# omarezz46/BayesDLL

Hardware: AMD Instinct MI355X
Metric: SG-HMC leapfrog steps/sec & HBM GB/s on ViT-L/32 params, 1/2/4/8 MI355X (higher is better)
Workload: dtype f32

## Files before the change

bayesdll_amd/_lib.py:

```python
from __future__ import annotations

import ctypes as C
import os
import threading

import numpy as np
import torch

HERE = os.path.dirname(os.path.abspath(__file__))
LIB_PATH = os.environ.get("BDL_SGMCMC_LIB", os.path.join(HERE, "libbdl_sgmcmc.so"))

BDL_OK = 0
CSGHMC, SGHMC, SGLD, SGHMC_GRAD, SGLD_GRAD, ADAM_SGHMC, ADAM_SGHMC_GRAD = range(7)
NOISE_NONE, NOISE_BUFFER, NOISE_PHILOX = 0, 1, 2
COLLECT_NONE, COLLECT_WELFORD_INIT, COLLECT_WELFORD, COLLECT_MEAN_INIT, COLLECT_MEAN = range(5)
MIX_BARE, MIX_PIPELINED, MIX_PACED = 0, 1, 2
ATTR_HEAD, ATTR_PRIOR, ATTR_SKIP, ATTR_GUNALIGNED = 0x1, 0x2, 0x4, 0x8
FLAG_FIRST_STEP, FLAG_RECIP_DIV, FLAG_MOMENTUM, FLAG_GRAD_READY = 0x1, 0x2, 0x4, 0x8
VAR_GIVEN, VAR_RAW_MOMENTS, VAR_WELFORD = 0, 1, 2
ABI_VERSION = 8

_fp = C.c_void_p


# ... 363 lines not shown


class MemberScore(C.Structure):
    _fields_ = [("n", C.c_int64), ("n_nonfinite", C.c_int64), ("n_wrong", C.c_int64),
                ("nll_sum", C.c_double)]


class MemberScoreArgs(C.Structure):
    _fields_ = [("logits", _fp), ("labels", _fp), ("scores", _fp), ("workspace", _fp),
                ("batch", C.c_int64), ("members", C.c_int32), ("groups", C.c_int32),
                ("classes", C.c_int32), ("grid_blocks", C.c_int32), ("flags", C.c_int32),
                ("pad0", C.c_int32)]


class MixtureTotals(C.Structure):
    _fields_ = [("n", C.c_int64), ("n_nonfinite", C.c_int64),
                ("expected_entropy_sum", C.c_double)]


class MixtureArgs(C.Structure):
    _fields_ = [("logits", _fp), ("weights", _fp), ("labels", _fp), ("logp", _fp),
                ("expected_entropy", _fp), ("totals", _fp), ("workspace", _fp),
                ("batch", C.c_int64), ("components", C.c_int32), ("draws", C.c_int32),
                ("groups", C.c_int32), ("classes", C.c_int32), ("combine", C.c_int32),
                ("grid_blocks", C.c_int32), ("flags", C.c_int32), ("pad0", C.c_int32)]


MIXTURE_EXPORTS = {
    "bdl_member_score_workspace_bytes": (C.c_int64, [C.c_int32, C.c_int32, C.c_int32]),
    "bdl_mixture_workspace_bytes": (C.c_int64, [C.c_int32, C.c_int32]),
    "bdl_member_score": (C.c_int, [C.POINTER(MemberScoreArgs), C.c_void_p]),
    "bdl_mixture": (C.c_int, [C.POINTER(MixtureArgs), C.c_void_p]),
}

RANK_U, RANK_ITILE, RANK_JTILE, RANK_MAX_ROWS = 2, 512, 1024, 65535
RANK_MAX_N = 2 ** 31 - 1


class RankTotals(C.Structure):
    _fields_ = [("n_pos", C.c_int64), ("n_neg", C.c_int64), ("n_excluded", C.c_int64),
                ("u2", C.c_int64), ("fp_at_tpr", C.c_int64), ("ap_sum", C.c_double)]


class RankArgs(C.Structure):
    _fields_ = [("scores", _fp), ("marks", _fp), ("ge_pos", _fp), ("ge_neg", _fp),
                ("gt_neg", _fp), ("totals", _fp), ("workspace", _fp), ("n", C.c_int64),
                ("need", C.c_int64), ("rows", C.c_int32), ("scores_per_group", C.c_int32),
                ("mark_rows", C.c_int32), ("tpr_num", C.c_int32), ("tpr_den", C.c_int32),
                ("pad0", C.c_int32)]


RANK_EXPORTS = {
    "bdl_rank_workspace_bytes": (C.c_int64, [C.c_int32, C.c_int64]),
    "bdl_rank": (C.c_int, [C.POINTER(RankArgs), C.c_void_p]),
}

DIVERSITY_MAX_VOTERS, DIVERSITY_MAX_CLASSES, DIVERSITY_WAVE_VOTERS = 64, 8192, 16
DIVERSITY_TILE, DIVERSITY_LDS_STRIDE, DIVERSITY_MAX_GRID = 64, 68, 1024
DIVERSITY_DEFAULT_WORKSPACE = 32 << 20
DIVERSITY_RESET = 0x1
DIVERSITY_INT_MATRICES = ("disagree", "both_wrong", "kl_unbounded")
DIVERSITY_SUM_MATRICES = ("tv_sum", "kl_sum")


def diversity_totals_dtype(voters):
    P = int(voters)
    return np.dtype([(k, np.int64) for k in ("n", "n_labelled", "n_nonfinite", "voters")]
                    + [(k, np.int64, (P, P)) for k in DIVERSITY_INT_MATRICES]
                    + [(k, np.float64, (P, P)) for k in DIVERSITY_SUM_MATRICES])


class DiversityArgs(C.Structure):
    _fields_ = [("logits", _fp), ("labels", _fp), ("totals", _fp), ("workspace", _fp),
                ("batch", C.c_int64), ("voters", C.c_int32), ("classes", C.c_int32),
                ("grid_blocks", C.c_int32), ("flags", C.c_int32)]


DIVERSITY_EXPORTS = {
    "bdl_diversity_totals_bytes": (C.c_int64, [C.c_int32]),
    "bdl_diversity_workspace_bytes": (C.c_int64, [C.c_int32, C.c_int32]),
    "bdl_diversity": (C.c_int, [C.POINTER(DiversityArgs), C.c_void_p]),
}

_lib = None
_lock = threading.Lock()


def lib():
    global _lib
    if _lib is not None:
        return _lib
    with _lock:
        if _lib is None:
            if not os.path.exists(LIB_PATH):
                raise RuntimeError(
                    f"bayesdll_amd: HIP library not found at {LIB_PATH}; build it with "
                    "`make -C bayesdll_amd/csrc` (or __graft_entry__.build()). There is no CPU "
                    "fallback for the fused SG-MCMC step.")
            h = C.CDLL(LIB_PATH)
            for name, (res, argt) in (list(EXPORTS.items()) + list(DIAG_EXPORTS.items())
                                      + list(CLIP_EXPORTS.items())
                                      + list(CHAIN_STEP_EXPORTS.items())
                                      + list(STATS_EXPORTS.items())
                                      + list(ESS_EXPORTS.items())
                                      + list(LOWP_EXPORTS.items())
                                      + list(LAYERS_EXPORTS.items())
                                      + list(PREDICT_EXPORTS.items())
                                      + list(FN_EXPORTS.items())
                                      + list(TEMPER_EXPORTS.items())
                                      + list(MIXTURE_EXPORTS.items())
                                      + list(RANK_EXPORTS.items())
                                      + list(DIVERSITY_EXPORTS.items())):
                fn = getattr(h, name)
                fn.restype = res
                fn.argtypes = argt
            if h.bdl_version() != ABI_VERSION:
                raise RuntimeError(f"bayesdll_amd: ABI version mismatch ({h.bdl_version()} != "
                                   f"{ABI_VERSION}); rebuild the library")
            _lib = h
    return _lib


def check(rc: int, what: str):
    if rc != BDL_OK:
        msg = lib().bdl_last_error().decode(errors="replace")
        raise RuntimeError(f"{what} failed (status {rc}): {msg}")
    return rc


def ptr(t):
    return None if t is None else C.c_void_p(t.data_ptr())


def current_stream_handle(device=None):
    return C.c_void_p(torch.cuda.current_stream(device).cuda_stream)


def require_hip(t: torch.Tensor, what: str):
    if not t.is_cuda:
        raise RuntimeError(f"bayesdll_amd: {what} must live on a HIP device (got {t.device}); "
                           "the fused SG-MCMC step has no CPU path")
    if t.dtype != torch.float32:
        raise RuntimeError(f"bayesdll_amd: {what} must be float32 (got {t.dtype})")
```

bayesdll_amd/csrc/bdl_api.hip:

```cpp
#include <algorithm>
#include "bdl_chain_common.hpp"
#include "bdl_measure.h"

#include <mutex>
#include <vector>

namespace bdl {
namespace {

thread_local std::string g_last_error;

int g_blocks_per_cu = 2;
int g_unroll = 1;
int g_grid_stride = 1;

int device_cu_count() {
  static int cached[64] = {0};
  int dev = 0;
  if (hipGetDevice(&dev) != hipSuccess || dev < 0 || dev >= 64) return 256;
  if (cached[dev] == 0) {
    int cus = 0;
    if (hipDeviceGetAttribute(&cus, hipDeviceAttributeMultiprocessorCount, dev) != hipSuccess ||
        cus <= 0)
      cus = 256;
    cached[dev] = cus;
  }
  return cached[dev];
}

constexpr int kMaxNormPartials = 2048;

template <int NOISE, bool RECIP, bool PRIOR>
__device__ __forceinline__ double sqnorm_fast(const KArgs& a, const StepConst& c, int64_t gb,
                                              float ns, double acc, const float* gp) {
  constexpr int U = 2;
  f4v th[U], g[U], t0[U], ep[U];
  const f4v z = {0.f, 0.f, 0.f, 0.f};
#pragma unroll
  for (int u = 0; u < U; ++u) {
    const int64_t e = (gb + (int64_t)u * kBlock + threadIdx.x) * 4;
    t0[u] = ep[u] = z;
    th[u] = vload(a.theta + e);
    g[u] = vload(gp + e);
    if constexpr (PRIOR) t0[u] = vload(a.prior_mean + e);
    if constexpr (NOISE == BDL_NOISE_BUFFER) ep[u] = vload(a.noise + e);
  }
#pragma unroll
  for (int u = 0; u < U; ++u) {
    const int64_t gi = gb + (int64_t)u * kBlock + threadIdx.x;
    if constexpr (NOISE == BDL_NOISE_PHILOX) ep[u] = step_noise4(a, gi);
#pragma unroll
    for (int j = 0; j < 4; ++j) {
      float xt = th[u][j], xg = g[u][j], xv = 0.f;
      update_core<BDL_SGLD_GRAD, NOISE, RECIP, PRIOR, false>(a, c, 0.f, ns, xt, xg, xv, t0[u][j],
                                                             ep[u][j]);
      acc = fma((double)xg, (double)xg, acc);
    }
  }
  return acc;
}

template <int NOISE, bool RECIP>
__device__ __forceinline__ void sqnorm_body(const KArgs& a, double* __restrict__ partials) {
  __shared__ double s_wave[kBlock / 64];
  constexpr int64_t kIter = (int64_t)kBlock * 2;
  StepConst c;
  c.sgd_mom = c.sgd_mom_read = c.has_m2 = c.grad_ready = c.clip = false;
  c.inv_s2 = a.inv_s2;
  c.inv_nd = a.inv_nd;
  c.inv_ca = c.inv_cb = c.clip_coef = 1.0f;
  const int64_t ngroups = (a.n + 3) >> 2, nfull = a.n >> 2;
  stage_runs(a);
  double acc = 0.0;
  int r = find_run_lds(a.nruns, (int64_t)blockIdx.x * kIter * 4);
  for (int64_t gb = (int64_t)blockIdx.x * kIter; gb < ngroups; gb += (int64_t)gridDim.x * kIter) {
    while (r < a.nruns - 1 && run_end(r) <= gb * 4) ++r;
    const int64_t gend = min(gb + kIter, ngroups);
    const uint32_t attr = run_attr(r);
    if (gend == gb + kIter && gend <= nfull && run_end(r) >= gend * 4 && !(attr & kNoFastPath)) {
      const float ns = (attr & BDL_ATTR_HEAD) ? a.ns1 : a.ns0;
      if (attr & BDL_ATTR_PRIOR)
        acc = sqnorm_fast<NOISE, RECIP, true>(a, c, gb, ns, acc, run_grad(a, r));
      else
        acc = sqnorm_fast<NOISE, RECIP, false>(a, c, gb, ns, acc, run_grad(a, r));
    } else {
// ... 406 lines not shown
  const int64_t per_iter = (int64_t)kBlock * unroll;
  const int64_t cap = (int64_t)device_cu_count() * g_blocks_per_cu;
  int64_t iters = (ngroups + per_iter - 1) / per_iter;
  int64_t grid = capped_grid(iters, cap);
  int64_t iters_per_block = (iters + grid - 1) / grid;
  grid = (iters + iters_per_block - 1) / iters_per_block;

  KArgs a;
  a.theta = s->theta;
  a.grad = s->grad;
  a.mom = s->mom;
  a.prior_mean = s->prior_mean;
  a.noise = s->noise;
  a.mom1 = s->mom1;
  a.mom2 = s->mom2;
  a.runs = s->runs;
  a.gbase = s->grad_base;
  a.nruns = s->nruns;
  a.flags = s->flags;
  a.n = s->n;
  a.groups_per_block = g_grid_stride ? 0 : iters_per_block * per_iter;
  a.lr0 = s->lr[0];
  a.lr1 = s->lr[1];
  a.ns0 = s->noise_scale[0];
  a.ns1 = s->noise_scale[1];
  a.one_minus_alpha = s->one_minus_alpha;
  a.prior_sig = s->prior_sig;
  a.sigma2 = s->sigma2;
  a.n_data = s->n_data;
  a.mu = s->mu;
  a.ca = s->collect_a;
  a.cb = s->collect_b;
  a.seed = s->seed;
  a.chain = s->chain;
  a.step = s->step;
  a.clip = clip;
  a.nonfinite = s->nonfinite;
  a.goff = s->philox_offset;
  a.cgroups = (uint32_t)s->chain_groups;
  a.inv_s2 = recip_or(s->inv_sigma2, s->sigma2);
  a.inv_nd = recip_or(s->inv_n_data, s->n_data);
  a.inv_ca = recip_or(s->inv_collect_a, s->collect_a);
  a.inv_cb = recip_or(s->inv_collect_b, s->collect_b);

  if (g_redirect_exec) {
    hipGraphNodeType nt = hipGraphNodeTypeEmpty;
    hipKernelNodeParams cur{};
    if (hipGraphNodeGetType(g_redirect_node, &nt) != hipSuccess || nt != hipGraphNodeTypeKernel ||
        hipGraphKernelNodeGetParams(g_redirect_node, &cur) != hipSuccess ||
        cur.func != (void*)k) {
      (void)hipGetLastError();
      return fail(BDL_ERR_ARG, "bdl_sgmcmc_step: the redirect node is not this step's kernel");
    }
    void* kp[] = {&a};
    hipKernelNodeParams p{};
    p.func = (void*)k;
    p.gridDim = dim3((unsigned)grid);
    p.blockDim = dim3(kBlock);
    p.sharedMemBytes = (unsigned)run_lds_bytes(s);
    p.kernelParams = kp;
    const hipError_t err = hipGraphExecKernelNodeSetParams(g_redirect_exec, g_redirect_node, &p);
    if (err != hipSuccess) {
      (void)hipGetLastError();
      g_last_error = std::string("bdl_sgmcmc_step: graph node update failed: ") +
                     hipGetErrorString(err);
      return BDL_ERR_LAUNCH;
    }
    return BDL_OK;
  }
  hipLaunchKernelGGL(k, dim3((unsigned)grid), dim3(kBlock), run_lds_bytes(s), stream, a);
  if (const int rc = launched("bdl_sgmcmc_step")) return rc;
  hipStreamCaptureStatus cs = hipStreamCaptureStatusNone;
  if (stream && hipStreamIsCapturing(stream, &cs) == hipSuccess &&
      cs == hipStreamCaptureStatusActive) {
    std::lock_guard<std::mutex> lk(g_captured_mu);
    if (std::find(g_captured_funcs.begin(), g_captured_funcs.end(), (const void*)k) ==
        g_captured_funcs.end())
      g_captured_funcs.push_back((const void*)k);
  }
  (void)hipGetLastError();
  return BDL_OK;
}


constexpr int kMixMaxR = 8, kMixMaxW = 6;
struct MixArgs {
  const float* r[kMixMaxR];
  float* w[kMixMaxW];
  int64_t n;
};

template <int NR, int U>
__device__ __forceinline__ void mix_load(const MixArgs& a, int64_t gb, f4v (&x)[U][NR]) {
#pragma unroll
  for (int u = 0; u < U; ++u) {
    const int64_t e = (gb + (int64_t)u * kBlock + threadIdx.x) * 4;
#pragma unroll
    for (int r = 0; r < NR; ++r) x[u][r] = vload(a.r[r] + e);
  }
}

template <int NR, int NW, int U, bool PACED>
__device__ __forceinline__ void mix_store(const MixArgs& a, int64_t gb, f4v (&x)[U][NR]) {
#pragma unroll
  for (int u = 0; u < U; ++u) {
    const int64_t gi = gb + (int64_t)u * kBlock + threadIdx.x;
    const int64_t e = gi * 4;
    f4v acc = x[u][0];
#pragma unroll
    for (int r = 1; r < NR; ++r) acc = acc + x[u][r] * 0.0f;
    if constexpr (PACED) acc = acc + philox_normal4((uint64_t)gi, 0x5eedull, 0, 1) * 0.0f;
#pragma unroll
    for (int w = 0; w < NW; ++w) vstore(a.w[w] + e, acc);
  }
}

template <int NR, int NW, int U, int S>
__global__ __launch_bounds__(kBlock) void bdl_mix_kernel(const MixArgs a) {
  constexpr int64_t kIter = (int64_t)kBlock * U;
  const int64_t ngroups = (a.n + 3) >> 2, nfull = a.n >> 2;
  const int64_t stride = (int64_t)gridDim.x * kIter;
  int64_t gb = (int64_t)blockIdx.x * kIter;
  if constexpr (S == BDL_MIX_PIPELINED) {
    f4v x[U][NR], y[U][NR];
    if (gb + kIter <= nfull) mix_load<NR, U>(a, gb, x);
    for (; gb + kIter <= nfull; gb += stride) {
      const bool more = gb + stride + kIter <= nfull;
      if (more) mix_load<NR, U>(a, gb + stride, y);
      mix_store<NR, NW, U, false>(a, gb, x);
      if (more) {
#pragma unroll
        for (int u = 0; u < U; ++u)
#pragma unroll
          for (int r = 0; r < NR; ++r) x[u][r] = y[u][r];
      }
    }
  } else {
    for (; gb + kIter <= nfull; gb += stride) {
      f4v x[U][NR];
      mix_load<NR, U>(a, gb, x);
      mix_store<NR, NW, U, S == BDL_MIX_PACED>(a, gb, x);
    }
  }
  if (gb < ngroups) {
    for (int u = 0; u < U; ++u) {
      const int64_t gi = gb + (int64_t)u * kBlock + threadIdx.x;
      if (gi >= ngroups) break;
      const int64_t e = gi * 4;
      f4v acc = ld4(a.r[0], e, a.n);
      for (int r = 1; r < NR; ++r) acc = acc + ld4(a.r[r], e, a.n) * 0.0f;
      for (int w = 0; w < NW; ++w) st4(a.w[w], e, a.n, acc);
    }
  }
}

typedef void (*MixKernel)(const MixArgs);

template <int NR, int NW, int S>
MixKernel pick_mix_u(int unroll) {
  switch (unroll) {
    case 1: return bdl_mix_kernel<NR, NW, 1, S>;
    case 4: return bdl_mix_kernel<NR, NW, 4, S>;
    default: return bdl_mix_kernel<NR, NW, 2, S>;
  }
}

template <int NR, int NW>
MixKernel pick_mix_s(int schedule, int unroll) {
  switch (schedule) {
    case BDL_MIX_BARE: return pick_mix_u<NR, NW, BDL_MIX_BARE>(unroll);
    case BDL_MIX_PIPELINED: return pick_mix_u<NR, NW, BDL_MIX_PIPELINED>(unroll);
    case BDL_MIX_PACED: return pick_mix_u<NR, NW, BDL_MIX_PACED>(unroll);
  }
  return nullptr;
}

MixKernel pick_mix(int nr, int nw, int schedule, int unroll) {
  if (nr == 2 && nw == 1) return pick_mix_s<2, 1>(schedule, unroll);
  if (nr == 3 && nw == 2) return pick_mix_s<3, 2>(schedule, unroll);
  if (nr == 4 && nw == 2) return pick_mix_s<4, 2>(schedule, unroll);
  if (nr == 3 && nw == 4) return pick_mix_s<3, 4>(schedule, unroll);
  if (nr == 5 && nw == 4) return pick_mix_s<5, 4>(schedule, unroll);
  if (nr == 7 && nw == 5) return pick_mix_s<7, 5>(schedule, unroll);
  return nullptr;
}

}

void set_last_error(const std::string& msg) { g_last_error = msg; }
bool graph_redirect_active() { return g_redirect_exec != nullptr; }
int cu_count() { return device_cu_count(); }

}

using namespace bdl;

extern "C" {

int bdl_version(void) { return BDL_ABI_VERSION; }

int bdl_graph_find_step_node(void* graph, const void* theta, int64_t n, void** node) {
  if (!graph || !node) return fail(BDL_ERR_NULL, "bdl_graph_find_step_node: null argument");
  *node = nullptr;
  std::vector<const void*> funcs;
  {
    std::lock_guard<std::mutex> lk(g_captured_mu);
    funcs = g_captured_funcs;
  }
  size_t count = 0;
  if (hipGraphGetNodes((hipGraph_t)graph, nullptr, &count) != hipSuccess) {
    (void)hipGetLastError();
    return fail(BDL_ERR_ARG, "bdl_graph_find_step_node: hipGraphGetNodes failed");
  }
  std::vector<hipGraphNode_t> nodes(count);
  if (count && hipGraphGetNodes((hipGraph_t)graph, nodes.data(), &count) != hipSuccess) {
    (void)hipGetLastError();
    return fail(BDL_ERR_ARG, "bdl_graph_find_step_node: hipGraphGetNodes failed");
  }
  int found = 0;
  for (hipGraphNode_t nd : nodes) {
    hipGraphNodeType t = hipGraphNodeTypeEmpty;
    if (hipGraphNodeGetType(nd, &t) != hipSuccess || t != hipGraphNodeTypeKernel) continue;
    hipKernelNodeParams p{};
    if (hipGraphKernelNodeGetParams(nd, &p) != hipSuccess) continue;
    if (std::find(funcs.begin(), funcs.end(), (const void*)p.func) == funcs.end()) continue;
    if (!p.kernelParams || !p.kernelParams[0]) continue;
    const KArgs* ka = (const KArgs*)p.kernelParams[0];
    if ((const void*)ka->theta == theta && ka->n == n) {
      *node = (void*)nd;
      ++found;
    }
  }
  (void)hipGetLastError();
  if (found != 1) {
    *node = nullptr;
    return fail(BDL_ERR_ARG, "bdl_graph_find_step_node: " + std::to_string(found) +
                                 " step nodes over this range");
  }
  return BDL_OK;
// ... 364 lines not shown
```

bayesdll_amd/flat.py:

```python
from __future__ import annotations

import contextlib
import ctypes as C

import numpy as np
import torch

from . import _lib as L
from .arena import default_grad_arena


def segment_attrs(names, readout_name, bias, requires_grad):
    attrs = []
    for nm, rg in zip(names, requires_grad):
        a = 0
        if readout_name is not None and readout_name in nm:
            a |= L.ATTR_HEAD
        if not ("bias" in nm and bias == "uninformative"):
            a |= L.ATTR_PRIOR
        if not rg:
            a |= L.ATTR_SKIP
        attrs.append(a)
    return attrs


def build_runs(offsets, numels, attrs, n):
    nseg = len(offsets)
    segs = (L.Segment * max(nseg, 1))()
    for i, (o, k, a) in enumerate(zip(offsets, numels, attrs)):
        segs[i].offset, segs[i].numel, segs[i].attr, segs[i].pad = int(o), int(k), int(a), 0
    cap = 2 * nseg + 2
    runs = (L.Run * cap)()
    nr = L.lib().bdl_build_runs(segs, nseg, int(n), runs, cap)
    if nr < 0:
        L.check(nr, "bdl_build_runs")
    out = torch.empty(nr, 2, dtype=torch.int64)
    for i in range(nr):
        out[i, 0] = runs[i].end
        out[i, 1] = runs[i].attr
    return out


GRAD_MODES = ("tensor", "flat")
MAX_TENSOR_RUNS = 2730
GRAD_TABLE_CACHE = 8


def default_grad_mode():
    import os
    m = os.environ.get("BDL_GRAD_MODE", "tensor")
    if m not in GRAD_MODES:
        raise ValueError(f"BDL_GRAD_MODE must be one of {GRAD_MODES}, got {m!r}")
    return m


COMPUTE_DTYPES = {None: None, "fp32": None, "float32": None, torch.float32: None,
                  "bf16": torch.bfloat16, "bfloat16": torch.bfloat16,
                  torch.bfloat16: torch.bfloat16}


def check_compute_dtype(compute_dtype):
    try:
        return COMPUTE_DTYPES[compute_dtype]
    except (KeyError, TypeError):
        raise ValueError(f"bayesdll_amd: compute_dtype must be fp32 or bf16, got "
                         f"{compute_dtype!r}") from None


def refuse_lowp_network(net, ntensors, grad_mode=None):
    if (grad_mode or default_grad_mode()) != "tensor":
        raise ValueError("bayesdll_amd: bf16 compute reads autograd's bf16 gradients in place: "
                         "the flat gradient vector (BDL_GRAD_MODE=flat) is not supported")
    if ntensors > MAX_TENSOR_RUNS:
        raise ValueError(f"bayesdll_amd: bf16 compute needs one run per tensor in the kernel's "
                         f"LDS table ({ntensors} parameter tensors > {MAX_TENSOR_RUNS}); the "
                         "flat gradient fallback is not supported")
    if default_grad_arena():
        raise ValueError("bayesdll_amd: bf16 compute does not support the gradient arena "
                         "(BDL_GRAD_ARENA=1)")
    fbuf = [nm for nm, b in net.named_buffers() if b.is_floating_point()]
    if fbuf:
        raise ValueError("bayesdll_amd: bf16 compute does not support networks with "
                         f"floating-point buffers (e.g. BatchNorm running statistics): {fbuf[:3]}")


class FlatState:

    def __init__(self, net, net0=None, *, readout_name=None, bias="informative",
                 need_prior=False, need_mom=True, need_noise=False, extra=(), grad_mode=None,
                 compute_dtype=None):
        named = list(net.named_parameters())
        if not named:
            raise ValueError("bayesdll_amd: the network has no parameters")
        self.compute_dtype = check_compute_dtype(compute_dtype)
        if self.compute_dtype is not None:
            refuse_lowp_network(net, len(named), grad_mode)
        self.names = [nm for nm, _ in named]
        self.params = [p for _, p in named]
        self.shapes = [tuple(p.shape) for p in self.params]
        self.numels = [p.numel() for p in self.params]
        self.offsets = np.concatenate([[0], np.cumsum(self.numels)[:-1]]).astype(np.int64).tolist()
        self.n = int(sum(self.numels))
        dev = self.params[0].device
        for nm, p in named:
            L.require_hip(p.data, f"parameter {nm!r}")
            if p.device != dev:
                raise RuntimeError("bayesdll_amd: all parameters must be on one device")
        self.device = dev
        self.readout_name = readout_name if readout_name is not None else getattr(
            net, "readout_name", None)
        self.bias = bias
        self.requires_grad = [p.requires_grad for p in self.params]
        self.grad_mode = grad_mode or default_grad_mode()
        if self.grad_mode not in GRAD_MODES:
            raise ValueError(f"grad_mode must be one of {GRAD_MODES}")
        if self.grad_mode == "tensor" and len(self.params) > MAX_TENSOR_RUNS:
            import warnings
            warnings.warn(f"bayesdll_amd: {len(self.params)} parameter tensors > "
                          f"{MAX_TENSOR_RUNS}: using the flat gradient vector")
            self.grad_mode = "flat"

        names_ = ["theta"] + (["grad"] if self.grad_mode == "flat" else []) + \
            (["mom"] if need_mom else []) + (["prior"] if need_prior else []) + list(extra)
        vecs = {nm: torch.zeros(self.n, dtype=torch.float32, device=dev) for nm in names_}
        self.extra = {nm: vecs[nm] for nm in extra}
        self.theta = vecs["theta"]
        with torch.no_grad():
            for p, o, k in zip(self.params, self.offsets, self.numels):
                self.theta[o:o + k].copy_(p.data.reshape(-1))
                p.data = self.theta[o:o + k].view(p.shape)
        self.shadow = None
        if self.compute_dtype is not None:
            self.shadow = torch.empty(self.n, dtype=self.compute_dtype, device=dev)
            self.refresh_shadow()
            for p, o, k in zip(self.params, self.offsets, self.numels):
                p.data = self.shadow[o:o + k].view(p.shape)
        self.grad = vecs["grad"].zero_() if self.grad_mode == "flat" else None
        self.gbase = None
        self._bind_grads()
        self.arena = None
        if self.grad_mode == "tensor" and default_grad_arena():
            from .arena import GradArena
            self.arena = GradArena(dev, 4 * self.n)

        self.mom = vecs["mom"].zero_() if need_mom else None
        self.prior = None
        if need_prior:
            self.prior = vecs["prior"].zero_()
            if net0 is not None:
                p0 = list(net0.parameters())
                if [tuple(q.shape) for q in p0] != self.shapes:
                    raise ValueError("bayesdll_amd: net0 does not match net's parameter shapes")
                with torch.no_grad():
                    for q, o, k in zip(p0, self.offsets, self.numels):
                        self.prior[o:o + k].copy_(q.detach().reshape(-1))
        self.noise = torch.empty(self.n, dtype=torch.float32, device=dev) if need_noise else None
        self.nonfinite = torch.zeros(1, dtype=torch.int32, device=dev)

        attrs = segment_attrs(self.names, self.readout_name, bias, self.requires_grad)
        self.attrs = attrs
        self.runs = build_runs(self.offsets, self.numels, attrs, self.n).to(dev)
        self.nruns = int(self.runs.shape[0])
        self._base_runs = (self.runs, self.nruns)
        self._skip_tables = {}
        self._grad_tables = {}
        self._untouched = ()
        self._touched = [False] * len(self.params) if self.grad_mode == "flat" else []
        self._hooks = [p.register_hook(self._mark(i))
                       for i, p in enumerate(self.params) if p.requires_grad] \
            if self.grad_mode == "flat" else []

    def _mark(self, i):
        touched = self._touched

        def hook(grad):
            if grad is not None:
                touched[i] = True
        return hook

    @classmethod
    def from_segments(cls, segments, readout_name, *, bias="informative", device="cuda",
                      need_prior=False, need_mom=True, need_noise=False, init=None, extra=()):
        self = cls.__new__(cls)
        self.names = [nm for nm, _ in segments]
        self.shapes = [tuple(s) for _, s in segments]
        self.numels = [int(np.prod(s)) for s in self.shapes]
        self.offsets = np.concatenate([[0], np.cumsum(self.numels)[:-1]]).astype(np.int64).tolist()
        self.n = int(sum(self.numels))
        self.device = torch.device(device)
        if self.device.type == "cuda" and self.device.index is None:
            self.device = torch.device("cuda", torch.cuda.current_device())
        self.readout_name = readout_name
        self.bias = bias
        self.requires_grad = [True] * len(self.names)
        self.params = []
        self._grad_ptrs = []
        f32 = dict(dtype=torch.float32, device=self.device)
        names_ = (["theta"] if init is None else []) + ["grad"] + (["mom"] if need_mom else []) \
            + (["prior"] if need_prior else []) + list(extra)
        vecs = {nm: torch.zeros(self.n, **f32) for nm in names_}
        self.extra = {nm: vecs[nm] for nm in extra}
        self.theta = vecs["theta"] if init is None else init
        self.grad_mode = "flat"
        self.compute_dtype = None
        self.shadow = None
        self.gbase = None
        self.arena = None
        self._grad_tables = {}
        self._untouched = ()
        self.grad = vecs["grad"].zero_()
        self.mom = vecs["mom"].zero_() if need_mom else None
        self.prior = vecs["prior"].zero_() if need_prior else None
        self.noise = torch.empty(self.n, **f32) if need_noise else None
        self.nonfinite = torch.zeros(1, dtype=torch.int32, device=self.device)
        self.attrs = segment_attrs(self.names, readout_name, bias, self.requires_grad)
        self.runs = build_runs(self.offsets, self.numels, self.attrs, self.n).to(self.device)
        self.nruns = int(self.runs.shape[0])
        self._base_runs = (self.runs, self.nruns)
        self._skip_tables = {}
        self._touched = []
        self._hooks = []
        return self

    def _bind_grads(self):
        if self.grad_mode == "tensor":
            for p in self.params:
                p.grad = None
            self._grad_ptrs = [0 if rg else None for rg in self.requires_grad]
            return
        self._grad_ptrs = []
        for p, o, k, rg in zip(self.params, self.offsets, self.numels,
                               [p.requires_grad for p in self.params]):
            if rg:
                p.grad = self.grad[o:o + k].view(p.shape)
                self._grad_ptrs.append(p.grad.data_ptr())
            else:
                self._grad_ptrs.append(None)

    def zero_grad(self):
        if self.grad_mode == "tensor":
            for p in self.params:
                p.grad = None
            return
        self.grad.zero_()
        for i in range(len(self._touched)):
            self._touched[i] = False
        for p, ptr in zip(self.params, self._grad_ptrs):
            if ptr is not None and (p.grad is None or p.grad.data_ptr() != ptr):
                self._bind_grads()
                break

    def backward_routing(self):
        if self.arena is None:
            return contextlib.nullcontext()
        return self.arena.routing()

    def sync_grads(self):
        if self.grad_mode == "tensor":
            self._sync_tensor_grads()
            return
        rebind = False
        untouched = []
        for i, (p, o, k, ptr) in enumerate(zip(self.params, self.offsets, self.numels,
                                               self._grad_ptrs)):
            if ptr is None:
                continue
            g = p.grad
            if g is None:
                self.grad[o:o + k].zero_()
                untouched.append(i)
                rebind = True
            else:
                if g.data_ptr() != ptr:
                    self.grad[o:o + k].copy_(g.reshape(-1))
                    rebind = True
                if self._touched and not self._touched[i]:
                    untouched.append(i)
        if rebind:
            self._bind_grads()
        self._select_runs(tuple(untouched))

    def _select_runs(self, untouched):
        if not untouched:
# ... 220 lines not shown
```

bayesdll_amd/kernels.py:

```python
from __future__ import annotations

import ctypes as C
import os

import numpy as np
import torch

from . import _lib as L
from . import ess as E

DIV_MODE = os.environ.get("BDL_DIV_MODE", "recip")


def _div_flag(div_mode=None):
    return L.FLAG_RECIP_DIV if (div_mode or DIV_MODE) == "recip" else 0


def _inv(s):
    s = float(s)
    return 1.0 / s if s != 0.0 else 0.0


def _step_args(state, method, *, lrs, noise_scale, noise_mode, one_minus_alpha=1.0,
               prior_sig=0.0, sigma2=1.0, n_data=1.0, mu=0.0, first_step=False,
# ... 1446 lines not shown
    a.scalars = scalars.data_ptr()
    a.n1, a.chain_groups, a.chains = int(state.n1), int(state.chain_groups), int(state.K)
    a.method, a.noise_mode, a.collect = int(method), int(noise_mode), int(collect)
    a.flags = ((L.FLAG_FIRST_STEP if first_step else 0) | (L.FLAG_MOMENTUM if momentum else 0)
               | _div_flag(div_mode))
    a.blocks_per_chain, a.unroll = int(blocks_per_chain), int(unroll)
    a.collect_a, a.collect_b = float(collect_a), float(collect_b)
    a.inv_collect_a, a.inv_collect_b = _inv(collect_a), _inv(collect_b)
    a.seed = int(seed) & 0xFFFFFFFFFFFFFFFF
    a.chain = int(chain) & 0xFFFFFFFFFFFFFFFF
    a.step = int(step) & 0xFFFFFFFFFFFFFFFF
    return a


def chain_step(state, method, *, scalars, **kw):
    K_ = int(state.K)
    if (scalars.dtype != torch.float32 or not scalars.is_cuda or not scalars.is_contiguous()
            or scalars.numel() != K_ * 12 or scalars.device != state.theta.device):
        raise ValueError("chain_step: scalars must be a contiguous float32 [K, 12] tensor on the "
                         "state's device")
    if not kw.get("blocks_per_chain"):
        kw["blocks_per_chain"] = chain_step_blocks_per_chain(state.n1, K_, state.theta.device,
                                                             kw.get("unroll") or 1)
    a = chain_step_args(state, method, scalars=scalars, **kw)
    dev = state.theta.device
    t = getattr(state, "timer", None)
    e0 = t.begin() if t is not None else None
    L.check(L.lib().bdl_chain_step(a, L.current_stream_handle(dev)), "bdl_chain_step")
    if e0 is not None:
        t.end(e0, alg_bytes_per_elem(a) * int(a.n1) * K_)


def philox_normal(n, seed, chain, step, device="cuda"):
    out = torch.empty(n, dtype=torch.float32, device=device)
    L.check(L.lib().bdl_philox_normal(out.data_ptr(), int(n), int(seed), int(chain), int(step),
                                      L.current_stream_handle(out.device)), "bdl_philox_normal")
    return out


_ACTIVE = [None]
LIBRARY_DEFAULT = (2, 1, 1)


def set_launch_config(blocks_per_cu=0, unroll=0, grid_stride=0):
    _ACTIVE[0] = (int(blocks_per_cu), int(unroll), int(grid_stride))
    return L.lib().bdl_set_launch_config(int(blocks_per_cu), int(unroll), int(grid_stride))


def restore_launch_config(packed):
    return set_launch_config((packed >> 8) & 0xFFFF, packed & 0xFF, (packed >> 24) & 0xFF)


def _use_geometry(state, kind="step"):
    cfg = getattr(state, {"collect": "collect_cfg", "init": "init_cfg"}.get(kind, "launch_cfg"),
                  None)
    if cfg is None:
        cfg = getattr(state, "launch_cfg", None)
    if cfg is not None and cfg != _ACTIVE[0]:
        set_launch_config(*cfg)


AUTOTUNE_CANDIDATES = ((2, 1, 1), (1, 4, 1), (3, 1, 1), (2, 4, 1), (1, 2, 1), (2, 2, 1))
AUTOTUNE_BY_METHOD = {
    "csghmc": AUTOTUNE_CANDIDATES + ((3, 4, 1), (1, 1, 1)),
    "sgld": AUTOTUNE_CANDIDATES + ((3, 4, 1), (4, 4, 1), (1, 1, 1)),
    "adam": AUTOTUNE_CANDIDATES + ((1, 1, 1), (4, 4, 1)),
}
_TUNED = {}
_TUNED_COLLECT = {}
COLLECT_EXTRA = ((1, 1, 1),)


ADAM_EXTRA = ("adam_m", "adam_v", "sgd_buf")


def _scratch_launcher(n, dev, method):
    return _scratch_launchers(n, dev, method)[0]


def _scratch_launchers(n, dev, method):
    from .flat import FlatState, moment_pair
    st = FlatState.from_segments([("w", (int(n),))], None, device=dev,
                                 need_prior=method != "csghmc",
                                 extra=ADAM_EXTRA if method == "adam" else ())
    st.theta.zero_()
    if method == "csghmc":
        kw = dict(lrs=(1e-4, 1e-4), noise_scale=(0.0, 0.0), noise_mode=L.NOISE_NONE,
                  one_minus_alpha=0.9, prior_sig=1.0)

        def launch():
            sgmcmc_step(st, L.CSGHMC, **kw)
    elif method == "sgld":
        st.prior.zero_()
        kw = dict(lrs=(1e-4, 1e-4), noise_scale=(1e-3, 1e-3), noise_mode=L.NOISE_PHILOX,
                  sigma2=1.0, n_data=1e6, mu=0.5, momentum=True)

        def launch():
            sgmcmc_step(st, L.SGLD, **kw)
    elif method == "adam":
        st.prior.zero_()
        m, v, buf = (st.extra[k] for k in ADAM_EXTRA)
        kw = dict(adam_m=m, adam_v=v, sgd_buf=buf, beta1=0.9, beta2=0.999, eps=1e-8, t=3,
                  momentum_decay=0.1, nd=0.01, lrs=(1e-4, 1e-4), noise_mode=L.NOISE_PHILOX,
                  sigma2=1.0, n_data=1e6, mu=0.5, momentum=True)

        def launch():
            adam_step(st, L.ADAM_SGHMC, **kw)
    else:
        raise ValueError(f"unknown method {method!r}")
    moms = []

    def launch_collect():
        if not moms:
            moms.extend(moment_pair(int(n), dev) if method == "csghmc" else
                        (torch.zeros_like(st.theta), torch.zeros_like(st.theta)))
            moms[0].copy_(st.theta)
            moms[1].zero_()
        if method == "csghmc":
            sgmcmc_step(st, L.CSGHMC, lrs=(1e-4, 1e-4), noise_scale=(1e-7, 1e-7),
                        noise_mode=L.NOISE_PHILOX, one_minus_alpha=0.9, prior_sig=1.0,
                        collect=L.COLLECT_WELFORD, mom1=moms[0], mom2=moms[1], collect_a=3.0)
        elif method == "sgld":
            sgmcmc_step(st, L.SGLD, collect=L.COLLECT_MEAN, mom1=moms[0], mom2=moms[1],
                        collect_a=2.0, collect_b=3.0, **kw)
        else:
            adam_step(st, L.ADAM_SGHMC, collect=L.COLLECT_MEAN, mom1=moms[0], mom2=moms[1],
                      collect_a=2.0, collect_b=3.0, **kw)
    return launch, launch_collect


def _device(device):
    return torch.device(device) if device is not None else torch.device(
        "cuda", torch.cuda.current_device())


def autotune(n, device=None, reps=6, candidates=None, method="csghmc", collect=False):
    import numpy as np
    dev = _device(device)
    if candidates is None:
        candidates = AUTOTUNE_BY_METHOD.get(method, AUTOTUNE_CANDIDATES)
    launch, launch_collect = _scratch_launchers(n, dev, method)

    def pick(fn, cands):
        times = measure(fn, cands, reps)
        top = sorted(times, key=times.get)[:3]
        again = measure(fn, top, 2 * reps)
        for cfg in top:
            times[cfg] = 0.5 * (times[cfg] + again[cfg])
        return min(top, key=times.get), times

    def measure(fn, cfgs, k):
        out = {}
        for cfg in cfgs:
            set_launch_config(*cfg)
            for _ in range(2):
                fn()
            ev = [(torch.cuda.Event(enable_timing=True), torch.cuda.Event(enable_timing=True))
                  for _ in range(k)]
            for e0, e1 in ev:
                e0.record()
                fn()
                e1.record()
            torch.cuda.synchronize(dev)
            out[cfg] = float(np.median([a.elapsed_time(b) for a, b in ev]))
        return out

    best, times = pick(launch, candidates)
# ... 111 lines not shown
```

Before: 927.0.

## Autotune physical placement of state vectors by timing candidate buffer assignments

```diff
diff --git a/bayesdll_amd/_lib.py b/bayesdll_amd/_lib.py
--- a/bayesdll_amd/_lib.py
+++ b/bayesdll_amd/_lib.py
@@ -469,6 +469,23 @@
     "bdl_diversity": (C.c_int, [C.POINTER(DiversityArgs), C.c_void_p]),
 }
 
+PLACE_MAX_CANDIDATES, PLACE_MAX_ASSIGNMENTS, PLACE_MAX_ROLES, PLACE_MAX_REPS = 16, 128, 4, 16
+PLACE_MARGIN = 0.045
+
+
+class PlaceArgs(C.Structure):
+    _fields_ = [("candidates", _fp), ("assignments", _fp), ("ms", _fp), ("n", C.c_int64),
+                ("window", C.c_int64), ("ncand", C.c_int32), ("nassign", C.c_int32),
+                ("nrmw", C.c_int32), ("nro", C.c_int32), ("blocks_per_cu", C.c_int32),
+                ("unroll", C.c_int32), ("reps", C.c_int32), ("launches", C.c_int32)]
+
+
+PLACE_EXPORTS = {
+    "bdl_place_times": (C.c_int, [C.POINTER(PlaceArgs), C.c_void_p]),
+    "bdl_place_choose": (C.c_int, [C.POINTER(C.c_float), C.POINTER(C.c_int32), C.c_int32,
+                                   C.c_int32, C.c_int32, C.c_int32, C.c_uint32]),
+}
+
 _lib = None
 _lock = threading.Lock()
 
@@ -497,7 +514,8 @@
                                       + list(TEMPER_EXPORTS.items())
                                       + list(MIXTURE_EXPORTS.items())
                                       + list(RANK_EXPORTS.items())
-                                      + list(DIVERSITY_EXPORTS.items())):
+                                      + list(DIVERSITY_EXPORTS.items())
+                                      + list(PLACE_EXPORTS.items())):
                 fn = getattr(h, name)
                 fn.restype = res
                 fn.argtypes = argt
diff --git a/bayesdll_amd/csrc/bdl_api.hip b/bayesdll_amd/csrc/bdl_api.hip
--- a/bayesdll_amd/csrc/bdl_api.hip
+++ b/bayesdll_amd/csrc/bdl_api.hip
@@ -1,6 +1,7 @@
 #include <algorithm>
 #include "bdl_chain_common.hpp"
 #include "bdl_measure.h"
+#include "bdl_mix.hpp"
 
 #include <mutex>
 #include <vector>
@@ -573,79 +574,6 @@
   return BDL_OK;
 }
 
-
-constexpr int kMixMaxR = 8, kMixMaxW = 6;
-struct MixArgs {
-  const float* r[kMixMaxR];
-  float* w[kMixMaxW];
-  int64_t n;
-};
-
-template <int NR, int U>
-__device__ __forceinline__ void mix_load(const MixArgs& a, int64_t gb, f4v (&x)[U][NR]) {
-#pragma unroll
-  for (int u = 0; u < U; ++u) {
-    const int64_t e = (gb + (int64_t)u * kBlock + threadIdx.x) * 4;
-#pragma unroll
-    for (int r = 0; r < NR; ++r) x[u][r] = vload(a.r[r] + e);
-  }
-}
-
-template <int NR, int NW, int U, bool PACED>
-__device__ __forceinline__ void mix_store(const MixArgs& a, int64_t gb, f4v (&x)[U][NR]) {
-#pragma unroll
-  for (int u = 0; u < U; ++u) {
-    const int64_t gi = gb + (int64_t)u * kBlock + threadIdx.x;
-    const int64_t e = gi * 4;
-    f4v acc = x[u][0];
-#pragma unroll
-    for (int r = 1; r < NR; ++r) acc = acc + x[u][r] * 0.0f;
-    if constexpr (PACED) acc = acc + philox_normal4((uint64_t)gi, 0x5eedull, 0, 1) * 0.0f;
-#pragma unroll
-    for (int w = 0; w < NW; ++w) vstore(a.w[w] + e, acc);
-  }
-}
-
-template <int NR, int NW, int U, int S>
-__global__ __launch_bounds__(kBlock) void bdl_mix_kernel(const MixArgs a) {
-  constexpr int64_t kIter = (int64_t)kBlock * U;
-  const int64_t ngroups = (a.n + 3) >> 2, nfull = a.n >> 2;
-  const int64_t stride = (int64_t)gridDim.x * kIter;
-  int64_t gb = (int64_t)blockIdx.x * kIter;
-  if constexpr (S == BDL_MIX_PIPELINED) {
-    f4v x[U][NR], y[U][NR];
-    if (gb + kIter <= nfull) mix_load<NR, U>(a, gb, x);
-    for (; gb + kIter <= nfull; gb += stride) {
-      const bool more = gb + stride + kIter <= nfull;
-      if (more) mix_load<NR, U>(a, gb + stride, y);
-      mix_store<NR, NW, U, false>(a, gb, x);
-      if (more) {
-#pragma unroll
-        for (int u = 0; u < U; ++u)
-#pragma unroll
-          for (int r = 0; r < NR; ++r) x[u][r] = y[u][r];
-      }
-    }
-  } else {
-    for (; gb + kIter <= nfull; gb += stride) {
-      f4v x[U][NR];
-      mix_load<NR, U>(a, gb, x);
-      mix_store<NR, NW, U, S == BDL_MIX_PACED>(a, gb, x);
-    }
-  }
-  if (gb < ngroups) {
-    for (int u = 0; u < U; ++u) {
-      const int64_t gi = gb + (int64_t)u * kBlock + threadIdx.x;
-      if (gi >= ngroups) break;
-      const int64_t e = gi * 4;
-      f4v acc = ld4(a.r[0], e, a.n);
-      for (int r = 1; r < NR; ++r) acc = acc + ld4(a.r[r], e, a.n) * 0.0f;
-      for (int w = 0; w < NW; ++w) st4(a.w[w], e, a.n, acc);
-    }
-  }
-}
-
-typedef void (*MixKernel)(const MixArgs);
 
 template <int NR, int NW, int S>
 MixKernel pick_mix_u(int unroll) {
diff --git a/bayesdll_amd/csrc/bdl_mix.hpp b/bayesdll_amd/csrc/bdl_mix.hpp
--- /dev/null
+++ b/bayesdll_amd/csrc/bdl_mix.hpp
@@ -0,0 +1,97 @@
+#pragma once
+#include "bdl_kernels.hpp"
+#include "bdl_measure.h"
+
+namespace bdl {
+
+constexpr int kMixMaxR = 8, kMixMaxW = 6;
+constexpr int kMixKeep = 3;
+struct MixArgs {
+  const float* r[kMixMaxR];
+  float* w[kMixMaxW];
+  int64_t n;
+};
+
+template <int NR, int U>
+__device__ __forceinline__ void mix_load(const MixArgs& a, int64_t gb, f4v (&x)[U][NR]) {
+#pragma unroll
+  for (int u = 0; u < U; ++u) {
+    const int64_t e = (gb + (int64_t)u * kBlock + threadIdx.x) * 4;
+#pragma unroll
+    for (int r = 0; r < NR; ++r) x[u][r] = vload(a.r[r] + e);
+  }
+}
+
+template <int NR, int NW, int U, int S>
+__device__ __forceinline__ void mix_store(const MixArgs& a, int64_t gb, f4v (&x)[U][NR]) {
+#pragma unroll
+  for (int u = 0; u < U; ++u) {
+    const int64_t gi = gb + (int64_t)u * kBlock + threadIdx.x;
+    const int64_t e = gi * 4;
+    if constexpr (S == kMixKeep) {
+      static_assert(NW <= NR, "KEEP: every written stream is a read stream");
+#pragma unroll
+      for (int w = 0; w < NW; ++w) vstore(a.w[w] + e, x[u][w]);
+#pragma unroll
+      for (int r = NW; r < NR; ++r) asm volatile("" ::"v"(x[u][r]));
+    } else {
+      f4v acc = x[u][0];
+#pragma unroll
+      for (int r = 1; r < NR; ++r) acc = acc + x[u][r] * 0.0f;
+      if constexpr (S == BDL_MIX_PACED)
+        acc = acc + philox_normal4((uint64_t)gi, 0x5eedull, 0, 1) * 0.0f;
+#pragma unroll
+      for (int w = 0; w < NW; ++w) vstore(a.w[w] + e, acc);
+    }
+  }
+}
+
+template <int NR, int NW, int U, int S>
+__global__ __launch_bounds__(kBlock) void bdl_mix_kernel(const MixArgs a) {
+  constexpr int64_t kIter = (int64_t)kBlock * U;
+  const int64_t ngroups = (a.n + 3) >> 2, nfull = a.n >> 2;
+  const int64_t stride = (int64_t)gridDim.x * kIter;
+  int64_t gb = (int64_t)blockIdx.x * kIter;
+  if constexpr (S == BDL_MIX_PIPELINED) {
+    f4v x[U][NR], y[U][NR];
+    if (gb + kIter <= nfull) mix_load<NR, U>(a, gb, x);
+    for (; gb + kIter <= nfull; gb += stride) {
+      const bool more = gb + stride + kIter <= nfull;
+      if (more) mix_load<NR, U>(a, gb + stride, y);
+      mix_store<NR, NW, U, BDL_MIX_BARE>(a, gb, x);
+      if (more) {
+#pragma unroll
+        for (int u = 0; u < U; ++u)
+#pragma unroll
+          for (int r = 0; r < NR; ++r) x[u][r] = y[u][r];
+      }
+    }
+  } else {
+    for (; gb + kIter <= nfull; gb += stride) {
+      f4v x[U][NR];
+      mix_load<NR, U>(a, gb, x);
+      mix_store<NR, NW, U, S>(a, gb, x);
+    }
+  }
+  if (gb < ngroups) {
+    for (int u = 0; u < U; ++u) {
+      const int64_t gi = gb + (int64_t)u * kBlock + threadIdx.x;
+      if (gi >= ngroups) break;
+      const int64_t e = gi * 4;
+      if constexpr (S == kMixKeep) {
+        f4v x[NR];
+        for (int r = 0; r < NR; ++r) x[r] = ld4(a.r[r], e, a.n);
+        for (int w = 0; w < NW; ++w) st4(a.w[w], e, a.n, x[w]);
+        for (int r = NW; r < NR; ++r) asm volatile("" ::"v"(x[r]));
+      } else {
+        f4v acc = ld4(a.r[0], e, a.n);
+        for (int r = 1; r < NR; ++r) acc = acc + ld4(a.r[r], e, a.n) * 0.0f;
+        for (int w = 0; w < NW; ++w) st4(a.w[w], e, a.n, acc);
+      }
+    }
+  }
+}
+
+typedef void (*MixKernel)(const MixArgs);
+
+}
diff --git a/bayesdll_amd/csrc/bdl_place.hip b/bayesdll_amd/csrc/bdl_place.hip
--- /dev/null
+++ b/bayesdll_amd/csrc/bdl_place.hip
@@ -0,0 +1,173 @@
+#include <cmath>
+
+#include "bdl_chain_common.hpp"
+#include "bdl_mix.hpp"
+#include "bdl_place.h"
+
+namespace bdl {
+namespace {
+
+template <int NR, int NW>
+MixKernel pick_keep_u(int unroll) {
+  switch (unroll) {
+    case 1: return bdl_mix_kernel<NR, NW, 1, kMixKeep>;
+    case 2: return bdl_mix_kernel<NR, NW, 2, kMixKeep>;
+    default: return bdl_mix_kernel<NR, NW, 4, kMixKeep>;
+  }
+}
+
+MixKernel pick_keep(int nrmw, int nro, int unroll) {
+  if (nrmw == 2 && nro == 1) return pick_keep_u<3, 2>(unroll);
+  if (nrmw == 2 && nro == 2) return pick_keep_u<4, 2>(unroll);
+  return nullptr;
+}
+
+bool row_ok(const int32_t* row, int nroles, int ncand) {
+  for (int i = 0; i < nroles; ++i) {
+    if (row[i] < 0 || row[i] >= ncand) return false;
+    for (int j = 0; j < i; ++j)
+      if (row[j] == row[i]) return false;
+  }
+  return true;
+}
+
+const char* table_error(const int32_t* assignments, int32_t nassign, int32_t nroles,
+                        int32_t ncand) {
+  if (!assignments) return "null assignments";
+  if (ncand < 2 || ncand > BDL_PLACE_MAX_CANDIDATES) return "ncand in [2, 16]";
+  if (nassign < 1 || nassign > BDL_PLACE_MAX_ASSIGNMENTS) return "nassign in [1, 128]";
+  if (nroles < 2 || nroles > BDL_PLACE_MAX_ROLES || nroles > ncand)
+    return "2 to 4 roles, at most one per candidate";
+  return nullptr;
+}
+
+struct Events {
+  hipEvent_t e[2 * BDL_PLACE_MAX_REPS] = {};
+  int n = 0;
+  bool create(int count) {
+    for (; n < count; ++n)
+      if (hipEventCreate(&e[n]) != hipSuccess) return false;
+    return true;
+  }
+  ~Events() {
+    for (int i = 0; i < n; ++i) (void)hipEventDestroy(e[i]);
+  }
+};
+
+}
+}
+
+using namespace bdl;
+
+extern "C" {
+
+int bdl_place_times(bdl_place_args* p, void* stream) {
+  if (const int rc = no_redirect("bdl_place_times")) return rc;
+  if (!p) return fail(BDL_ERR_NULL, "bdl_place_times: null args");
+  p->launches = 0;
+  if (!p->candidates || !p->ms) return fail(BDL_ERR_NULL, "bdl_place_times: null candidates / ms");
+  const int nroles = p->nrmw + p->nro;
+  if (p->nrmw != 2 || (p->nro != 1 && p->nro != 2))
+    return fail(BDL_ERR_ARG, "bdl_place_times: role patterns 2 + 1 and 2 + 2 (nrmw + nro)");
+  if (const char* e = table_error(p->assignments, p->nassign, nroles, p->ncand))
+    return fail(p->assignments ? BDL_ERR_ARG : BDL_ERR_NULL, std::string("bdl_place_times: ") + e);
+  if (p->n < 0 || p->window < 0 || p->n > INT64_MAX / 4)
+    return fail(BDL_ERR_ARG, "bdl_place_times: n and window >= 0");
+  if (p->blocks_per_cu < 1 || p->blocks_per_cu > 16 ||
+      (p->unroll != 1 && p->unroll != 2 && p->unroll != 4))
+    return fail(BDL_ERR_ARG, "bdl_place_times: blocks_per_cu in [1, 16], unroll 1, 2 or 4");
+  if (p->reps < 1 || p->reps > BDL_PLACE_MAX_REPS)
+    return fail(BDL_ERR_ARG, "bdl_place_times: reps in [1, 16]");
+  const float* base[BDL_PLACE_MAX_CANDIDATES];
+  int64_t len = p->n;
+  for (int i = 0; i < p->ncand; ++i) {
+    const void* c = p->candidates[i];
+    if (!c) return fail(BDL_ERR_NULL, "bdl_place_times: null candidate");
+    if (misaligned(c, 3)) return fail(BDL_ERR_ALIGN, "bdl_place_times: candidate not 4-B aligned");
+    for (int j = 0; j < i; ++j)
+      if (overlap(c, p->candidates[j], 4 * (uint64_t)p->n, 4 * (uint64_t)p->n))
+        return fail(BDL_ERR_ARG, "bdl_place_times: candidates overlap");
+    const int64_t skip = (int64_t)((16 - (reinterpret_cast<uintptr_t>(c) & 15)) & 15) / 4;
+    base[i] = static_cast<const float*>(c) + skip;
+    len = std::min(len, p->n - skip);
+  }
+  for (int r = 0; r < p->nassign; ++r) {
+    if (!row_ok(p->assignments + (int64_t)r * nroles, nroles, p->ncand))
+      return fail(BDL_ERR_ARG, "bdl_place_times: an assignment's indices must be distinct "
+                  "candidates");
+    p->ms[r] = 0.0f;
+  }
+  if (p->window > 0) len = std::min(len, p->window);
+  if (len <= 0) return BDL_OK;
+
+  MixKernel k = pick_keep(p->nrmw, p->nro, p->unroll);
+  const int64_t per = (int64_t)kBlock * p->unroll;
+  const int grid = (int)capped_grid(block_iters(len, per), (int64_t)cu_count() * p->blocks_per_cu);
+  Events ev;
+  if (!ev.create(2 * p->reps)) {
+    (void)hipGetLastError();
+    return fail(BDL_ERR_LAUNCH, "bdl_place_times: hipEventCreate failed");
+  }
+  hipStream_t s = (hipStream_t)stream;
+  for (int r = 0; r < p->nassign; ++r) {
+    const int32_t* row = p->assignments + (int64_t)r * nroles;
+    MixArgs a{};
+    for (int i = 0; i < nroles; ++i) a.r[i] = base[row[i]];
+    for (int i = 0; i < p->nrmw; ++i) a.w[i] = const_cast<float*>(base[row[i]]);
+    a.n = len;
+    hipLaunchKernelGGL(k, dim3(grid), dim3(kBlock), 0, s, a);
+    ++p->launches;
+    bool recorded = true;
+    for (int t = 0; t < p->reps && recorded; ++t) {
+      recorded = hipEventRecord(ev.e[2 * t], s) == hipSuccess;
+      hipLaunchKernelGGL(k, dim3(grid), dim3(kBlock), 0, s, a);
+      ++p->launches;
+      recorded = recorded && hipEventRecord(ev.e[2 * t + 1], s) == hipSuccess;
+    }
+    if (const int rc = launched("bdl_place_times")) return rc;
+    if (!recorded) return fail(BDL_ERR_LAUNCH, "bdl_place_times: hipEventRecord failed");
+    if (hipEventSynchronize(ev.e[2 * p->reps - 1]) != hipSuccess) {
+      (void)hipGetLastError();
+      return fail(BDL_ERR_LAUNCH, "bdl_place_times: waiting for the timed launches failed");
+    }
+    float best = 0.0f;
+    for (int t = 0; t < p->reps; ++t) {
+      float ms = 0.0f;
+      if (hipEventElapsedTime(&ms, ev.e[2 * t], ev.e[2 * t + 1]) != hipSuccess) {
+        (void)hipGetLastError();
+        return fail(BDL_ERR_LAUNCH, "bdl_place_times: hipEventElapsedTime failed");
+      }
+      if (t == 0 || ms < best) best = ms;
+    }
+    p->ms[r] = best;
+  }
+  return BDL_OK;
+}
+
+int bdl_place_choose(const float* ms, const int32_t* assignments, int32_t nassign, int32_t nroles,
+                     int32_t ncand, int32_t default_row, uint32_t fixed_roles) {
+  if (!ms) return fail(BDL_ERR_NULL, "bdl_place_choose: null ms");
+  if (const char* e = table_error(assignments, nassign, nroles, ncand))
+    return fail(assignments ? BDL_ERR_ARG : BDL_ERR_NULL, std::string("bdl_place_choose: ") + e);
+  if (default_row < 0 || default_row >= nassign)
+    return fail(BDL_ERR_ARG, "bdl_place_choose: default_row not a row of the table");
+  const int32_t* def = assignments + (int64_t)default_row * nroles;
+  if (!row_ok(def, nroles, ncand)) return default_row;
+  for (int r = 0; r < nassign; ++r)
+    if (!std::isfinite(ms[r]) || !(ms[r] > 0.0f)) return default_row;
+  const float bound = ms[default_row] * (1.0f - BDL_PLACE_MARGIN);
+  int best = default_row;
+  for (int r = 0; r < nassign; ++r) {
+    if (r == default_row) continue;
+    const int32_t* row = assignments + (int64_t)r * nroles;
+    if (!row_ok(row, nroles, ncand)) continue;
+    bool moved_fixed = false;
+    for (int i = 0; i < nroles; ++i)
+      if (((fixed_roles >> i) & 1u) && row[i] != def[i]) moved_fixed = true;
+    if (moved_fixed || !(ms[r] < bound)) continue;
+    if (best == default_row || ms[r] < ms[best]) best = r;
+  }
+  return best;
+}
+
+}
diff --git a/bayesdll_amd/flat.py b/bayesdll_amd/flat.py
--- a/bayesdll_amd/flat.py
+++ b/bayesdll_amd/flat.py
@@ -88,7 +88,7 @@
 
     def __init__(self, net, net0=None, *, readout_name=None, bias="informative",
                  need_prior=False, need_mom=True, need_noise=False, extra=(), grad_mode=None,
-                 compute_dtype=None):
+                 compute_dtype=None, place=None):
         named = list(net.named_parameters())
         if not named:
             raise ValueError("bayesdll_amd: the network has no parameters")
@@ -123,6 +123,7 @@
         names_ = ["theta"] + (["grad"] if self.grad_mode == "flat" else []) + \
             (["mom"] if need_mom else []) + (["prior"] if need_prior else []) + list(extra)
         vecs = {nm: torch.zeros(self.n, dtype=torch.float32, device=dev) for nm in names_}
+        vecs = self._place(vecs, extra, place)
         self.extra = {nm: vecs[nm] for nm in extra}
         self.theta = vecs["theta"]
         with torch.no_grad():
@@ -170,6 +171,21 @@
                        for i, p in enumerate(self.params) if p.requires_grad] \
             if self.grad_mode == "flat" else []
 
+    def _place(self, vecs, extra, enabled, fixed=()):
+        from . import placement
+        if extra:
+            self.placement = {"spares": 0, "moved": [],
+                              "skipped": "extra vectors: another step pattern"}
+            self.tuned = {"placement": self.placement}
+            return vecs
+        rmw = [nm for nm in ("theta", "mom") if nm in vecs]
+        ro = [nm for nm in ("grad", "prior") if nm in vecs]
+        vecs, rec = placement.place(vecs, rmw, ro, fixed=fixed, device=self.device,
+                                    enabled=enabled)
+        self.placement = rec
+        self.tuned = {"placement": rec}
+        return vecs
+
     def _mark(self, i):
         touched = self._touched
 
@@ -180,7 +196,8 @@
 
     @classmethod
     def from_segments(cls, segments, readout_name, *, bias="informative", device="cuda",
-                      need_prior=False, need_mom=True, need_noise=False, init=None, extra=()):
+                      need_prior=False, need_mom=True, need_noise=False, init=None, extra=(),
+                      place=None):
         self = cls.__new__(cls)
         self.names = [nm for nm, _ in segments]
         self.shapes = [tuple(s) for _, s in segments]
@@ -199,6 +216,15 @@
         names_ = (["theta"] if init is None else []) + ["grad"] + (["mom"] if need_mom else []) \
             + (["prior"] if need_prior else []) + list(extra)
         vecs = {nm: torch.zeros(self.n, **f32) for nm in names_}
+        if init is None:
+            vecs = self._place(vecs, extra, place)
+        elif (init.dtype == torch.float32 and init.device == self.device and init.is_contiguous()
+              and init.numel() == self.n):
+            vecs = self._place({"theta": init, **vecs}, extra, place, fixed=("theta",))
+        else:
+            self.placement = {"spares": 0, "moved": [],
+                              "skipped": "init is not a flat fp32 vector on the device"}
+            self.tuned = {"placement": self.placement}
         self.extra = {nm: vecs[nm] for nm in extra}
         self.theta = vecs["theta"] if init is None else init
         self.grad_mode = "flat"
diff --git a/bayesdll_amd/kernels.py b/bayesdll_amd/kernels.py
--- a/bayesdll_amd/kernels.py
+++ b/bayesdll_amd/kernels.py
@@ -1552,7 +1552,7 @@
     from .flat import FlatState, moment_pair
     st = FlatState.from_segments([("w", (int(n),))], None, device=dev,
                                  need_prior=method != "csghmc",
-                                 extra=ADAM_EXTRA if method == "adam" else ())
+                                 extra=ADAM_EXTRA if method == "adam" else (), place=False)
     st.theta.zero_()
     if method == "csghmc":
         kw = dict(lrs=(1e-4, 1e-4), noise_scale=(0.0, 0.0), noise_mode=L.NOISE_NONE,
diff --git a/bayesdll_amd/placement.py b/bayesdll_amd/placement.py
--- /dev/null
+++ b/bayesdll_amd/placement.py
@@ -0,0 +1,146 @@
+from __future__ import annotations
+
+import ctypes as C
+import itertools
+import os
+import time
+
+import torch
+
+from . import _lib as L
+
+SPARES_DEFAULT = 2
+MIN_ELEMS_DEFAULT = 1 << 26
+SPARE_FRACTION = 0.25
+WINDOW_ELEMS = 1 << 27
+REPS = 3
+GEOMETRY = (1, 4)
+
+_HOOK = {"times": None, "reps": None}
+
+
+def spares_requested():
+    v = os.environ.get("BDL_PLACE_SPARES", str(SPARES_DEFAULT))
+    try:
+        k = int(v)
+    except ValueError:
+        raise ValueError(f"BDL_PLACE_SPARES must be an integer >= 0, got {v!r}") from None
+    if k < 0 or k > L.PLACE_MAX_CANDIDATES - 4:
+        raise ValueError(f"BDL_PLACE_SPARES must be in [0, {L.PLACE_MAX_CANDIDATES - 4}], got {k}")
+    return k
+
+
+def min_elems():
+    return int(os.environ.get("BDL_PLACE_MIN_ELEMS", str(MIN_ELEMS_DEFAULT)))
+
+
+def assignments_for(nstate, ncand, nrmw, nro, fixed):
+    nroles = nrmw + nro
+    default = tuple(range(nroles))
+    rows = [default]
+    free_rmw = [r for r in range(nrmw) if r not in fixed]
+    for pair in itertools.combinations(range(ncand), nrmw):
+        if any(pair[r] != default[r] for r in range(nrmw) if r in fixed):
+            continue
+        if not free_rmw and pair != default[:nrmw]:
+            continue
+        row = list(pair)
+        left = [c for c in range(ncand) if c not in pair]
+        for r in range(nrmw, nroles):
+            c = default[r] if default[r] in left else left[0]
+            left.remove(c)
+            row.append(c)
+        if tuple(row) not in rows:
+            rows.append(tuple(row))
+        if len(rows) == L.PLACE_MAX_ASSIGNMENTS:
+            break
+    return rows
+
+
+def probe(cands, n, rows, nrmw, nro, stream, window=WINDOW_ELEMS, reps=REPS, geometry=GEOMETRY):
+    nroles = nrmw + nro
+    ptrs = (C.c_void_p * len(cands))(*[c.data_ptr() for c in cands])
+    flat = (C.c_int32 * (len(rows) * nroles))(*[c for row in rows for c in row])
+    ms = (C.c_float * len(rows))()
+    a = L.PlaceArgs()
+    a.candidates = C.cast(ptrs, C.c_void_p)
+    a.assignments = C.cast(flat, C.c_void_p)
+    a.ms = C.cast(ms, C.c_void_p)
+    a.n, a.window, a.ncand, a.nassign = int(n), int(window), len(cands), len(rows)
+    a.nrmw, a.nro, a.blocks_per_cu, a.unroll, a.reps = nrmw, nro, geometry[0], geometry[1], reps
+    L.check(L.lib().bdl_place_times(a, stream), "bdl_place_times")
+    return list(ms), int(a.launches)
+
+
+def choose(ms, rows, ncand, fixed=()):
+    nroles = len(rows[0])
+    t = (C.c_float * len(rows))(*ms)
+    flat = (C.c_int32 * (len(rows) * nroles))(*[c for row in rows for c in row])
+    mask = sum(1 << r for r in fixed)
+    rc = L.lib().bdl_place_choose(t, flat, len(rows), nroles, ncand, 0, mask)
+    if rc < 0:
+        L.check(rc, "bdl_place_choose")
+    return rc
+
+
+def place(vecs, rmw, ro, *, fixed=(), device, enabled=None):
+    out, rec = _place(vecs, rmw, ro, fixed=fixed, device=device, enabled=enabled)
+    if os.environ.get("BDL_PLACE_VERBOSE") == "1":
+        import json
+        import sys
+        print("bdl_place " + json.dumps(rec), file=sys.stderr, flush=True)
+    return out, rec
+
+
+def _place(vecs, rmw, ro, *, fixed=(), device, enabled=None):
+    t0 = time.perf_counter()
+    rec = {"spares": 0, "moved": []}
+    if enabled is False:
+        return vecs, {**rec, "skipped": "disabled by the caller"}
+    if torch.device(device).type != "cuda":
+        return vecs, {**rec, "skipped": "not a HIP device"}
+    want = spares_requested()
+    if want == 0:
+        return vecs, {**rec, "skipped": "BDL_PLACE_SPARES=0"}
+    n = int(vecs[rmw[0]].numel()) if rmw else 0
+    if len(rmw) != 2 or len(ro) > 2:
+        return vecs, {**rec, "skipped": "no step pattern with two read-modify-write vectors"}
+    if n < max(1, min_elems()):
+        return vecs, {**rec, "skipped": f"{n} elements per vector < {min_elems()}: "
+                                        "the Infinity Cache can hold one"}
+    free, _ = torch.cuda.mem_get_info(device)
+    k = min(want, int(SPARE_FRACTION * free) // max(4 * n, 1))
+    if k == 0:
+        return vecs, {**rec, "skipped": f"no spare of {4 * n >> 20} MiB within "
+                                        f"{SPARE_FRACTION:g} x free {free >> 20} MiB"}
+    roles = list(rmw) + list(ro)
+    nro = max(1, len(ro))
+    spares = [torch.zeros(n, dtype=torch.float32, device=device) for _ in range(k)]
+    cands = [vecs[r] for r in roles] + spares
+    rows = assignments_for(len(roles), len(cands), 2, nro,
+                           {roles.index(f) for f in fixed if f in roles})
+    rec.update(spares=k, roles=roles, assignments=[list(r) for r in rows],
+               transient_bytes=4 * n * k)
+    stream = L.current_stream_handle(device)
+    try:
+        if _HOOK["times"] is not None:
+            ms, launches = [float(x) for x in _HOOK["times"](rows)], 0
+        else:
+            ms, launches = probe(cands, n, rows, 2, nro, stream,
+                                 reps=REPS if _HOOK["reps"] is None else _HOOK["reps"])
+        best = choose(ms, rows, len(cands), {roles.index(f) for f in fixed if f in roles})
+    except RuntimeError as e:
+        del spares, cands
+        rec.update(error=str(e), chosen=list(rows[0]), launches=0,
+                   ms_total=round((time.perf_counter() - t0) * 1e3, 3))
+        return vecs, rec
+    out = dict(vecs)
+    for i, r in enumerate(roles):
+        if rows[best][i] != i:
+            out[r] = cands[rows[best][i]]
+            rec["moved"].append(r)
+    del spares, cands
+    rec.update(ms=[round(x, 4) for x in ms], chosen=list(rows[best]), chosen_row=best,
+               launches=launches, margin=L.PLACE_MARGIN,
+               ms_total=round((time.perf_counter() - t0) * 1e3, 3))
+    return out, rec
diff --git a/include/bdl_place.h b/include/bdl_place.h
--- /dev/null
+++ b/include/bdl_place.h
@@ -0,0 +1,44 @@
+#ifndef BDL_PLACE_H
+#define BDL_PLACE_H
+
+#include <stdint.h>
+
+#include "bdl_sgmcmc.h"
+
+#ifdef __cplusplus
+extern "C" {
+#endif
+
+#define BDL_PLACE_MAX_CANDIDATES 16
+#define BDL_PLACE_MAX_ASSIGNMENTS 128
+#define BDL_PLACE_MAX_ROLES 4
+#define BDL_PLACE_MAX_REPS 16
+
+#define BDL_PLACE_MARGIN 0.045f
+
+typedef struct bdl_place_args {
+  const void* const* candidates;
+  const int32_t* assignments;
+  float* ms;
+  int64_t n;
+  int64_t window;
+  int32_t ncand;
+  int32_t nassign;
+  int32_t nrmw;
+  int32_t nro;
+  int32_t blocks_per_cu;
+  int32_t unroll;
+  int32_t reps;
+  int32_t launches;
+} bdl_place_args;
+
+int bdl_place_times(bdl_place_args* args, void* hip_stream);
+
+int bdl_place_choose(const float* ms, const int32_t* assignments, int32_t nassign, int32_t nroles,
+                     int32_t ncand, int32_t default_row, uint32_t fixed_roles);
+
+#ifdef __cplusplus
+}
+#endif
+
+#endif
```

After: 928.1 (median of 3 runs). No clear change (+0.1%).
